# oxfordcontrol/COSMO.jl

Hardware: NVIDIA H100
Metric: ADMM iterations/sec (higher is better)
Workload: dtype f64

## Files before the change

cosmo.jl_b200/csrc/common.cuh:

```cuda
#pragma once
#include <cuda_runtime.h>
#include <stdint.h>

#include <limits>

namespace cosmo {

constexpr int kBlock = 256;
constexpr int kWarpsPerBlock = kBlock / 32;
constexpr int kMaxGrid = 132 * 8;
constexpr int kMaxRed = 8;

template <typename T>
struct CsrView {
  const int* rowptr;
  const int* col;
  const T* val;
};

template <typename T>
struct RedBuf {
  T* partials;
  T* out;
  unsigned* ticket;
// ... 39 lines not shown
}
__device__ __forceinline__ void mbar_wait(uint64_t* bar, unsigned parity) {
  const unsigned addr = (unsigned)__cvta_generic_to_shared(bar);
  asm volatile(
      "{\n\t"
      ".reg .pred p;\n\t"
      "WAIT_LOOP:\n\t"
      "mbarrier.try_wait.parity.shared::cta.b64 p, [%0], %1;\n\t"
      "@p bra WAIT_DONE;\n\t"
      "bra WAIT_LOOP;\n\t"
      "WAIT_DONE:\n\t"
      "}" ::"r"(addr),
      "r"(parity)
      : "memory");
}

constexpr int kMaxRanks = 8;
template <typename T>
struct P2pView {
  T* peer_data[kMaxRanks];
  unsigned* peer_flags[kMaxRanks];
  const unsigned* local_flags;
  unsigned* seq;
  size_t stride;
  int nranks, rank;
};
__device__ __forceinline__ void st_release_sys(unsigned* p, unsigned v) {
  asm volatile("st.release.sys.global.u32 [%0], %1;" ::"l"(p), "r"(v) : "memory");
}
__device__ __forceinline__ unsigned ld_acquire_sys(const unsigned* p) {
// ... 111 lines not shown
```

cosmo.jl_b200/csrc/engine.cu:

```cuda
#include <cuda_runtime.h>
#include <dlfcn.h>
#include <math.h>
#include <stdio.h>
#include <stdlib.h>
#include <string.h>

#include <algorithm>
#include <functional>
#include <thread>
#include <chrono>
#include <string>
#include <vector>

#include "../../include/cosmo_b200.h"
#include "common.cuh"
#include "host.cuh"
#include "psd.cuh"
#include "cone3.cuh"
#include "aa.cuh"
#include "spmv.cuh"
#include "vector_kernels.cuh"
#include "ruiz.cuh"
#include "cg_persistent.cuh"
#include "ldl.cuh"
// ... 232 lines not shown
  std::vector<int> ldl_fptr_h_, ldl_bptr_h_;
  int ldl_N_ = 0, ldl_ws_ctas_ = 1, ldl_solve_nodes_ = 0, ldl_factor_nodes_ = 0;
  long long ldl_nnzK_ = 0, ldl_nnzL_ = 0, ldl_factorizations_ = 0;
  double ldl_symbolic_s_ = 0.0, ldl_factor_s_ = 0.0;
  DevBuf<int64_t> ldl_Kp_, ldl_Ksp_, ldl_Ksrc_, ldl_Lp_, ldl_Rp_, ldl_Rmap_;
  DevBuf<int> ldl_Ki_, ldl_Li_, ldl_Rj_, ldl_fcols_, ldl_fptr_, ldl_bcols_, ldl_bptr_, ldl_perm_, ldl_flags_;
  DevBuf<T> ldl_Kx_, ldl_Lx_, ldl_Rx_, ldl_D_, ldl_Dinv_, ldl_ws_, ldl_y_;
  GraphExec ldl_factor_graph_, ldl_solve_graph_;
  Event ldl_ev_[2];
  void ldl_setup();
  void ldl_factor();
  void ldl_solve();
  void destroy_ldl_factor_graph() { ldl_factor_graph_.reset(); }
  long long kkt_counter_ = 1;
  int last_cg_iters_ = 1;
  long long total_inner_ = 0, total_mults_ = 0;
  DevBuf<T> vec_m_, vec_n_, vec_n2_, dy_, dx_, ypart_;
  DevBuf<unsigned> chunk_ticket_;
  int num_sms_ = 132;
  DevBuf<T> sc_;
  DevBuf<int> isc_;
  DevBuf<T> partials_;
  DevBuf<unsigned> ticket_;
  PinnedBuf<T> h_sc_;
  PinnedBuf<int> h_isc_;
  cudaStream_t stream_ = nullptr;
  Event ev0_, ev1_;
  long long launches_ = 0;
  int nranks_ = 1, rank_ = 0;
  NcclComm comm_ = nullptr;
// ... 26 lines not shown
    cudaError_t e = cudaGetLastError();
    if (e != cudaSuccess) throw EngineError{COSMO_B200_ERR_CUDA, std::string("launch of ") + what + " failed: " + cudaGetErrorString(e)};
    ++launches_;
  }
  void sync() { CUDA_TRY(cudaStreamSynchronize(stream_)); }
  void upload_vec(DevBuf<T>& dst, const void* host, size_t count);
  void download_vec(void* host, const T* src, size_t count);
  void build_csr(DevCsr<T>& dst, const HostCsr& h);
  void build_windows(DevCsr<T>& dst, const HostCsr& h);
  void classify_and_set_rho(bool reset_rho, bool rebuild_vec = true);
  void allreduce_sum(T* buf, size_t count);
  void allreduce_max(T* buf, size_t count);

  template <typename Epi>
  void launch_spmv(const DevCsr<T>& M1, const T* x1, const DevCsr<T>* M2, const T* x2, int nrows, const Epi& epi,
                   RedBuf<T> rb, const char* name);
  void project_device(const T* w, bool with_rhs, const T* ws_rhs);
  void soc_norms(const T* ws, T* norm_out);
  void kkt_core(bool fused_tail, const T* w_src, T* w_dst);
  void kkt_op_stage2(const int* done, const T* u, const T* t_in, T* c_out, bool exchange = false);
  void kkt_cg(const int* done);
  void kkt_minres(bool full);
  void set_maxit(int v);
  void compute_residuals(const T* x, const T* s, const T* mu, bool ignore_scaling, double out[5]);
  bool adapt_rho(const T* x);
  bool primal_infeasible();
  bool dual_infeasible();
  double inf_rec_[8] = {0, 0, 0, 0, 0, 0, 0, 0};
  void recover_mu(const T* w_prev) {
    recover_mu_kernel<T><<<vgrid(m_), kBlock, 0, stream_>>>(m_, rho_vec_.p, w_prev + n_, s_.p, mu_.p);
    check_launch("recover_mu");
  }
  void read_scalars(int first, int count) {
    CUDA_TRY(cudaMemcpyAsync(h_sc_.p + first, sc_.p + first, count * sizeof(T), cudaMemcpyDeviceToHost, stream_));
    sync();
  }
// ... 709 lines not shown
    xv_.peer_data[r] = static_cast<T*>(pd);
    xv_.peer_flags[r] = static_cast<unsigned*>(pf);
  }
  for (int r = nranks; r < kMaxRanks; ++r) { xv_.peer_data[r] = nullptr; xv_.peer_flags[r] = nullptr; }
  xv_.local_flags = xchg_flags_.p;
  xv_.seq = xchg_seq_.p;
  xv_.nranks = nranks;
  xv_.rank = rank_;
  destroy_cg_graphs();
  p2p_ = true;
}

template <typename T>
template <typename Epi>
void Engine<T>::launch_spmv(const DevCsr<T>& M1, const T* x1, const DevCsr<T>* M2, const T* x2, int nrows,
                            const Epi& epi, RedBuf<T> rb, const char* name) {
  const CsrView<T> v2 = M2 ? M2->view() : CsrView<T>{nullptr, nullptr, nullptr};
  if (M1.windowed) {
    const size_t smem = (size_t)M1.W * sizeof(T);
    static bool configured[64] = {false};
    const int dev_slot = device_ & 63;
    if (!configured[dev_slot] || device_ >= 64) {
      CUDA_TRY(cudaFuncSetAttribute(spmv_win_kernel<T, Epi>, cudaFuncAttributeMaxDynamicSharedMemorySize, 204800));
      configured[dev_slot] = true;
    }
    spmv_win_kernel<T, Epi><<<M1.nctas, kWinThreads, smem, stream_>>>(M1.wview(), x1, v2, x2, epi, rb, ypart_.p,
                                                                      chunk_ticket_.p);
    check_launch(name);
    return;
  }
  const int lanes = M1.lanes;
  const int grid = sgrid(nrows, lanes);
  if (lanes == 32) spmv_kernel<T, 32, Epi><<<grid, kBlock, 0, stream_>>>(M1.view(), x1, v2, x2, nrows, epi, rb);
  else if (lanes == 8) spmv_kernel<T, 8, Epi><<<grid, kBlock, 0, stream_>>>(M1.view(), x1, v2, x2, nrows, epi, rb);
  else spmv_kernel<T, 2, Epi><<<grid, kBlock, 0, stream_>>>(M1.view(), x1, v2, x2, nrows, epi, rb);
  check_launch(name);
}

template <typename T>
void Engine<T>::soc_norms(const T* ws, T* norm_out) {
  if (!n_soc_) return;
  if (n_soc_chunks_) {
    soc_chunk_kernel<T><<<n_soc_chunks_, kBlock, 0, stream_>>>(ws, soc_chunk_start_.p, soc_chunk_len_.p, soc_chunk_sum_.p);
    check_launch("soc_chunk");
  }
  soc_final_kernel<T><<<(n_soc_ + 127) / 128, 128, 0, stream_>>>(soc_chunk_sum_.p, soc_cone_chunk_ptr_.p, n_soc_, norm_out);
  check_launch("soc_final");
}

template <typename T>
void Engine<T>::project_device(const T* w, bool with_rhs, const T* ws_rhs) {
// ... 10 lines not shown
  a.soc = SocTable<T>{soc_off_.p, soc_norm_.p};
  a.s = s_.p; a.ls = ls_.p; a.t0 = t0_.p; a.sigma = (T)st_.sigma;
  a.do_proj = 1; a.do_rhs = with_rhs ? 1 : 0;
  launch_proj_rhs(a);
}

template <typename T>
void Engine<T>::kkt_op_stage2(const int* done, const T* u, const T* t_in, T* c_out, bool exchange) {
  const bool lead = (rank_ == 0);
  const bool px = exchange && p2p_;
  const T sig = lead ? (T)st_.sigma : (T)0;
  const DevCsr<T>* M2 = nullptr;
  const T* pu = nullptr;
  if (At_.windowed) {
    if (lead && P_.nnz > 0) {
      launch_spmv(P_, u, (const DevCsr<T>*)nullptr, (const T*)nullptr, n_, EpiStore<T>{done, vec_n2_.p}, red(SC_TMP0), "spmv_P");
      pu = vec_n2_.p;
    }
  } else if (lead) {
    M2 = &P_;
  }
  launch_spmv(At_, t_in, M2, u, n_, EpiKktOp<T>{done, c_out, u, sig, pu}, red_ptr(cb_.p + n_), "spmv_kkt_op");
  if (px) {
    if (c_out != cb_.p) throw EngineError{COSMO_B200_ERR_INVALID, "peer exchange expects the operator output in cb_"};
    const int len = n_ + 1;
    const int gx = std::max(1, std::min(16, (len * (int)sizeof(T) + 32767) / 32768));
    p2p_push_kernel<T><<<dim3(gx, nranks_), kBlock, 0, stream_>>>(xv_, cb_.p, len, done, xchg_arrive_.p);
    check_launch("p2p_push");
  }
}

template <typename T>
void Engine<T>::set_maxit(int v) {
  if (cur_maxit_ == v) return;
  h_isc_[ISC_MAXIT] = v;
  CUDA_TRY(cudaMemcpyAsync(isc_.p + ISC_MAXIT, h_isc_.p + ISC_MAXIT, sizeof(int), cudaMemcpyHostToDevice, stream_));
  sync();
  cur_maxit_ = v;
}

template <typename T>
void Engine<T>::kkt_core(bool fused_tail, const T* w_src, T* w_dst) {
  const bool lead = (rank_ == 0);
  const bool full = (st_.kkt_solver == COSMO_B200_KKT_MINRES);
  const bool direct = (st_.kkt_solver == COSMO_B200_KKT_LDL);
  if (st_.kkt_solver != COSMO_B200_KKT_CG && st_.kkt_solver != COSMO_B200_KKT_MINRES_REDUCED && !full && !direct)
    throw EngineError{COSMO_B200_ERR_UNSUPPORTED, "unknown kkt_solver"};
  if (full && nranks_ > 1)
    throw EngineError{COSMO_B200_ERR_UNSUPPORTED, "full-KKT MINRES is single-GPU in this build (use CG or reduced MINRES when sharded)"};
  if (full || direct) {
    if (direct) ldl_solve();
    else kkt_minres(true);
    if (fused_tail) {
      admm_tail_kernel<T><<<vgrid(m_), kBlock, 0, stream_>>>(m_, nu_.p, rho_vec_.p, s_.p, w_src + n_, w_dst + n_, (T)st_.alpha);
      check_launch("admm_tail");
    }
    return;
  }
  launch_spmv(At_, t0_.p, (const DevCsr<T>*)nullptr, (const T*)nullptr, n_,
              EpiAddVec<T>{nullptr, rhsb_.p, lead ? ls_.p : nullptr}, red(SC_TMP0), "spmv_rhs");
  allreduce_sum(rhsb_.p, n_);
  if (st_.kkt_solver == COSMO_B200_KKT_CG) kkt_cg(isc_.p + ISC_DONE);
  else kkt_minres(false);
  kkt_counter_ += 1;
  if (fused_tail) {
    launch_spmv(A_, xsol_.p, (const DevCsr<T>*)nullptr, (const T*)nullptr, m_,
                EpiAdmmTail<T>{nullptr, ls_.p + n_, rho_vec_.p, s_.p, w_src + n_, w_dst + n_, (T)st_.alpha}, red(SC_TMP0),
                "spmv_admm_tail");
  } else {
    launch_spmv(A_, xsol_.p, (const DevCsr<T>*)nullptr, (const T*)nullptr, m_,
                EpiY2<T>{nullptr, nu_.p, ls_.p + n_, rho_vec_.p}, red(SC_TMP0), "spmv_y2");
  }
}

template <typename T>
void Engine<T>::kkt_cg(const int* done) {
  set_maxit(n_);
  if (persistent_cg_ok()) {
    launch_persistent_cg(st_.tol_constant / pow((double)kkt_counter_, st_.tol_exponent));
    return;
  }
  launch_spmv(A_, xsol_.p, (const DevCsr<T>*)nullptr, (const T*)nullptr, m_, EpiScale<T>{nullptr, tm_.p, rho_vec_.p},
              red(SC_TMP0), "spmv_A_scale");
  kkt_op_stage2(nullptr, xsol_.p, tm_.p, cb_.p, true);
  if (!p2p_) allreduce_sum(cb_.p, n_ + 1);
  const double tol_num = st_.tol_constant / pow((double)kkt_counter_, st_.tol_exponent);
  cg_init_kernel<T><<<vgrid(n_), kBlock, 0, stream_>>>(n_, rhsb_.p, cb_.p, r_.p, u_.p, red(SC_RES2),
                                                      CgInitFin<T>{sc_.p, isc_.p, (T)tol_num, p2p_ ? xchg_seq_.p : nullptr}, p2p_, xv_);
  check_launch("cg_init");
  if (!cg_graph_[0]) build_cg_graphs(done);
  int chunk = std::max(last_cg_iters_, 0);
  for (;;) {
    int left = chunk;
    for (int b = 3; b >= 0; --b)
      while (left >= (1 << b)) {
        CUDA_TRY(cudaGraphLaunch(cg_graph_[b], stream_));
        launches_ += (long long)(1 << b) * (At_.windowed && P_.nnz > 0 ? 5 : 4);
        left -= (1 << b);
      }
    CUDA_TRY(cudaMemcpyAsync(h_isc_.p, isc_.p, 2 * sizeof(int), cudaMemcpyDeviceToHost, stream_));
    sync();
    if (h_isc_[ISC_DONE]) break;
    chunk = 1;
  }
  const int iters = h_isc_[ISC_IT];
  last_cg_iters_ = iters;
  total_inner_ += iters;
  total_mults_ += 1 + iters;
}

template <typename T>
bool Engine<T>::persistent_cg_ok() {
// ... 25 lines not shown
  a.A = A_.view(); a.At = At_.view(); a.P = P_.view();
  a.n = n_; a.m = m_;
  a.rhs = rhsb_.p; a.rho = rho_vec_.p; a.x = xsol_.p; a.r = r_.p; a.u = u_.p; a.tm = tm_.p; a.c = cb_.p;
  a.partA = persist_part_.p; a.partB = persist_part_.p + (size_t)persist_grid_ * 2;
  a.sc = sc_.p; a.isc = isc_.p; a.sigma = (T)st_.sigma; a.tol_num = (T)tol_num;
  void* args[] = {&a};
  const void* fn = persist_lanes_ == 32 ? (const void*)cg_persistent_kernel<T, 32>
                 : persist_lanes_ == 8 ? (const void*)cg_persistent_kernel<T, 8> : (const void*)cg_persistent_kernel<T, 2>;
  CUDA_TRY(cudaLaunchCooperativeKernel(fn, dim3(persist_grid_), dim3(kBlock), args, 0, stream_));
  check_launch("cg_persistent");
  ++persist_solves_;
}

template <typename T>
void Engine<T>::cg_iteration_launches(const int* done) {
  cg_update_u_kernel<T><<<vgrid(n_), kBlock, 0, stream_>>>(n_, r_.p, u_.p, sc_.p, isc_.p);
  check_launch("cg_update_u");
  launch_spmv(A_, u_.p, (const DevCsr<T>*)nullptr, (const T*)nullptr, m_, EpiScale<T>{done, tm_.p, rho_vec_.p}, red(SC_TMP0),
              "spmv_A_scale");
  kkt_op_stage2(done, u_.p, tm_.p, cb_.p, true);
  if (!p2p_) allreduce_sum(cb_.p, n_ + 1);
  cg_update_xr_kernel<T><<<vgrid(n_), kBlock, 0, stream_>>>(n_, u_.p, cb_.p, cb_.p + n_, xsol_.p, r_.p, sc_.p, isc_.p, red(SC_RES2),
                                                         CgStepFin<T>{sc_.p, isc_.p, p2p_ ? xchg_seq_.p : nullptr}, p2p_, xv_);
  check_launch("cg_update_xr");
}

template <typename T>
void Engine<T>::build_cg_graphs(const int* done) {
  cg_iteration_launches(done);
  sync();
  const long long saved = launches_;
  for (int b = 0; b < 4; ++b)
    capture_graph(cg_graph_[b], stream_, [&] { for (int i = 0; i < (1 << b); ++i) cg_iteration_launches(done); });
  launches_ = saved;
}

template <typename T>
void Engine<T>::kkt_minres(bool full) {
// ... 86 lines not shown
  out[2] = nmax(nmax(m1, m2), m3);
  out[3] = nmax(nmax(d1, d2), d3);
  out[4] = (1.0 / c_) * (0.5 * xPx + qx);
}

template <typename T>
bool Engine<T>::adapt_rho(const T* x) {
  double r[5];
  compute_residuals(x, s_.p, mu_.p, true, r);
  double rp = r[0] / (r[2] + 1e-10);
  double rd = r[1] / (r[3] + 1e-10);
  double new_rho = rho_ * sqrt(rp / (rd + 1e-10));
  new_rho = std::min(std::max(new_rho, st_.RHO_MIN), st_.RHO_MAX);
  if (new_rho > st_.adaptive_rho_tolerance * rho_ || new_rho < (1.0 / st_.adaptive_rho_tolerance) * rho_) {
    rho_ = new_rho;
    rho_vec_kernel<T><<<vgrid(m_), kBlock, 0, stream_>>>(m_, rho_class_.p, (T)rho_, (T)st_.RHO_EQ_OVER_RHO_INEQ, (T)st_.RHO_MIN, rho_vec_.p);
    check_launch("rho_vec");
    ldl_dirty_ = true;
    rho_updates_.push_back(new_rho);
    return true;
  }
  return false;
}

template <typename T>
bool Engine<T>::primal_infeasible() {
  const T eps = (T)st_.eps_prim_inf;
  double* rec = inf_rec_;
  for (int k = 0; k < 8; ++k) rec[k] = (k == 0 || k >= 6) ? 0.0 : NAN;
  rec[1] = 1;
// ... 276 lines not shown

template <typename T>
void Engine<T>::accelerator_stats(int64_t* out) {
  out[0] = aa_accelerated_; out[1] = aa_declined_; out[2] = aa_rejected_;
  out[3] = aa_rho_restarts_; out[4] = aa_mem_restarts_; out[5] = aa_activated_at_;
}

template <typename T>
void Engine<T>::solve(cosmo_b200_result* out) {
  const double t_start = now_s();
  CUDA_TRY(cudaSetDevice(device_));
  const int n = n_, m = m_;
  const long long launches0 = launches_;
  total_inner_ = 0; total_mults_ = 0;
  persist_solves_ = 0;
  CUDA_TRY(cudaMemsetAsync(isc_.p + ISC_TOTAL, 0, sizeof(int), stream_));
  int status = COSMO_B200_UNDETERMINED;
  double cost = INFINITY;
  double info[5] = {INFINITY, INFINITY, 0.0, 0.0, INFINITY};
  long long iter = 0;
  bool rho_update_due = false, infeasibility_check_due = false;
  double res_time = 0.0;

  cur_ = 0; prev_ = 1;
  CUDA_TRY(cudaMemcpyAsync(W_[cur_].p, xs_.p, n * sizeof(T), cudaMemcpyDeviceToDevice, stream_));
  ws_from_mu_kernel<T><<<vgrid(m), kBlock, 0, stream_>>>(m, rho_vec_.p, mu_.p, s_.p, W_[cur_].p + n);
  check_launch("ws_from_mu");
  is_optimized_ = true;
  {
    const bool timers = (st_.verbose & 2) != 0 || (long long)n + m >= 20000 || !psd_.large_h.empty();
// ... 198 lines not shown
void Engine<T>::project(const void* ws, void* s_out) {
  CUDA_TRY(cudaSetDevice(device_));
  if (proj_w_.n < (size_t)n_ + m_) { proj_w_.alloc((size_t)n_ + m_); proj_s_.alloc(std::max(m_, 1), false); }
  upload_vec(vec_m_, ws, m_);
  CUDA_TRY(cudaMemcpyAsync(proj_s_.p, s_.p, m_ * sizeof(T), cudaMemcpyDeviceToDevice, stream_));
  CUDA_TRY(cudaMemcpyAsync(proj_w_.p + n_, vec_m_.p, m_ * sizeof(T), cudaMemcpyDeviceToDevice, stream_));
  project_device(proj_w_.p, false, nullptr);
  download_vec(s_out, s_.p, m_);
  CUDA_TRY(cudaMemcpyAsync(s_.p, proj_s_.p, m_ * sizeof(T), cudaMemcpyDeviceToDevice, stream_));
  sync();
}

template <typename T>
void Engine<T>::kkt_solve(const void* rhs, void* sol, int64_t* inner) {
  CUDA_TRY(cudaSetDevice(device_));
  upload_vec(ls_, rhs, (size_t)n_ + m_);
  scale_kernel<T><<<vgrid(m_), kBlock, 0, stream_>>>(m_, rho_vec_.p, ls_.p + n_, t0_.p);
  check_launch("scale_x2");
  kkt_core(false, nullptr, nullptr);
  download_vec(sol, xsol_.p, n_);
  download_vec(static_cast<T*>(sol) + n_, nu_.p, m_);
  sync();
  if (inner && st_.kkt_solver == COSMO_B200_KKT_LDL) {
    *inner = 0;
  } else if (inner) {
    CUDA_TRY(cudaMemcpyAsync(h_isc_.p, isc_.p, 2 * sizeof(int), cudaMemcpyDeviceToHost, stream_));
    sync();
    *inner = h_isc_[ISC_IT];
  }
}
// ... 152 lines not shown
template <typename T>
void Engine<T>::spmv(int which, const void* x, void* y) {
  CUDA_TRY(cudaSetDevice(device_));
  if (which == 0) {
    upload_vec(dx_, x, n_);
    launch_spmv(A_, dx_.p, (const DevCsr<T>*)nullptr, (const T*)nullptr, m_, EpiStore<T>{nullptr, vec_m_.p}, red(SC_TMP0), "spmv_A");
    download_vec(y, vec_m_.p, m_);
  } else if (which == 1) {
    upload_vec(dy_, x, m_);
    launch_spmv(At_, dy_.p, (const DevCsr<T>*)nullptr, (const T*)nullptr, n_, EpiStore<T>{nullptr, vec_n_.p}, red(SC_TMP0), "spmv_At");
    download_vec(y, vec_n_.p, n_);
  } else if (which == 2) {
    upload_vec(dx_, x, n_);
    launch_spmv(P_, dx_.p, (const DevCsr<T>*)nullptr, (const T*)nullptr, n_, EpiStore<T>{nullptr, vec_n_.p}, red(SC_TMP0), "spmv_P");
    download_vec(y, vec_n_.p, n_);
  } else {
    throw EngineError{COSMO_B200_ERR_INVALID, "spmv: which must be 0 (A), 1 (A') or 2 (P)"};
  }
  sync();
}

template <typename T>
void Engine<T>::spmv_bench(int which, int reps, double* ms, double* bytes) {
  CUDA_TRY(cudaSetDevice(device_));
  if (reps < 1) reps = 1;
  auto one = [&]() {
    if (which == 0)
      launch_spmv(A_, xsol_.p, (const DevCsr<T>*)nullptr, (const T*)nullptr, m_, EpiScale<T>{nullptr, tm_.p, rho_vec_.p}, red(SC_TMP0), "spmv_A_scale");
    else if (which == 1)
      launch_spmv(At_, tm_.p, (const DevCsr<T>*)nullptr, (const T*)nullptr, n_, EpiStore<T>{nullptr, vec_n_.p}, red(SC_TMP0), "spmv_At");
    else if (which == 2)
      launch_spmv(P_, xsol_.p, (const DevCsr<T>*)nullptr, (const T*)nullptr, n_, EpiStore<T>{nullptr, vec_n_.p}, red(SC_TMP0), "spmv_P");
// ... 286 lines not shown
```

cosmo.jl_b200/csrc/host.cuh:

```cuda
#pragma once
#include <cuda_runtime.h>
#include <stdio.h>

#include <string>
#include <vector>

#include "../../include/cosmo_b200.h"

namespace cosmo {

struct EngineError {
  int code;
  std::string msg;
};

#define CUDA_TRY(expr)                                                                              \
  do {                                                                                              \
    cudaError_t _e = (expr);                                                                        \
    if (_e != cudaSuccess) {                                                                        \
      char _b[512];                                                                                 \
      snprintf(_b, sizeof(_b), "CUDA error %s at %s:%d: %s", cudaGetErrorName(_e), __FILE__,        \
               __LINE__, cudaGetErrorString(_e));                                                   \
      throw EngineError{COSMO_B200_ERR_CUDA, _b};                                                   \
    }                                                                                               \
// ... 47 lines not shown
  cudaEvent_t e = nullptr;
  Event() {} Event(const Event&) = delete; Event& operator=(const Event&) = delete;
  ~Event() { if (e) cudaEventDestroy(e); }
  void create() { if (!e) CUDA_TRY(cudaEventCreate(&e)); }
  operator cudaEvent_t() const { return e; }
};

struct GraphExec {
  cudaGraphExec_t g = nullptr;
  GraphExec() {} GraphExec(const GraphExec&) = delete; GraphExec& operator=(const GraphExec&) = delete;
  ~GraphExec() { reset(); }
  void reset() { if (g) cudaGraphExecDestroy(g); g = nullptr; }
  operator cudaGraphExec_t() const { return g; }
};

template <typename F>
void capture_graph(GraphExec& out, cudaStream_t st, F&& launches) {
  out.reset();
  cudaGraph_t graph = nullptr;
  CUDA_TRY(cudaStreamBeginCapture(st, cudaStreamCaptureModeThreadLocal));
  launches();
  CUDA_TRY(cudaStreamEndCapture(st, &graph));
  CUDA_TRY(cudaGraphInstantiate(&out.g, graph, 0));
  CUDA_TRY(cudaGraphDestroy(graph));
}

}
```

cosmo.jl_b200/csrc/spmv.cuh:

```cuda
#pragma once
#include "common.cuh"

namespace cosmo {

template <typename T, bool NC>
__device__ __forceinline__ T gather_ld(const T* p) {
  if (NC) return __ldg(p);
  return __ldcg(p);
}

template <typename T, int LANES, bool NC = true>
__device__ __forceinline__ T row_partial(const CsrView<T>& M, const T* __restrict__ x, int row, int lane) {
  const int start = __ldg(M.rowptr + row);
  const int end = __ldg(M.rowptr + row + 1);
  T s0 = 0, s1 = 0;
  if (LANES == 32) {
    int a0 = (start + 3) & ~3;
    if (a0 > end) a0 = end;
    {
      const int i = start + lane;
      if (i < a0) s0 += __ldcs(M.val + i) * gather_ld<T, NC>(x + __ldcs(M.col + i));
    }
    const int body_end = a0 + ((end - a0) & ~3);
#pragma unroll 2
// ... 14 lines not shown
    for (int j = start + lane; j < end; j += LANES) s0 += __ldcs(M.val + j) * gather_ld<T, NC>(x + __ldcs(M.col + j));
  }
  return s0 + s1;
}

template <typename T, int LANES>
__device__ __forceinline__ T group_sum(T v) {
#pragma unroll
  for (int o = LANES / 2; o > 0; o >>= 1) v += __shfl_xor_sync(0xffffffffu, v, o, LANES);
  return v;
}

template <typename T, int LANES, typename Epi>
__global__ void __launch_bounds__(kBlock) spmv_kernel(CsrView<T> M1, const T* __restrict__ x1, CsrView<T> M2,
                                                      const T* __restrict__ x2, int nrows, Epi epi, RedBuf<T> rb) {
  if (epi.done != nullptr && *epi.done) return;
  constexpr int GROUPS = kBlock / LANES;
  const int lane = threadIdx.x % LANES;
  const int group = threadIdx.x / LANES;
  const int total_groups = gridDim.x * GROUPS;
  T accS[Epi::NS > 0 ? Epi::NS : 1];
  T accM[Epi::NM > 0 ? Epi::NM : 1];
#pragma unroll
  for (int k = 0; k < (Epi::NS > 0 ? Epi::NS : 1); ++k) accS[k] = 0;
#pragma unroll
  for (int k = 0; k < (Epi::NM > 0 ? Epi::NM : 1); ++k) accM[k] = 0;

  for (int base = blockIdx.x * GROUPS; base < nrows; base += total_groups) {
    const int row = base + group;
    const bool valid = row < nrows;
// ... 39 lines not shown
__device__ __forceinline__ T win_row_rest(const unsigned short* __restrict__ col, const T* __restrict__ val, const T* xs,
                                          int start, int end, int lane) {
  T s = 0;
  for (int j0 = start + 256; j0 < end; j0 += 256) {
    const int L = min(32, (end - j0) >> 3);
    if (lane < L) {
      const uint4 c = __ldcs(reinterpret_cast<const uint4*>(col + j0 + lane * 8));
      T v[8];
      load8_coalesced(val + j0, L, lane, v);
      s += win_fma8<T>(v, c, xs);
    }
  }
  return s;
}

template <typename T, typename Epi>
__global__ void __launch_bounds__(kWinThreads, 1) spmv_win_kernel(WcsrView<T> M, const T* __restrict__ x, CsrView<T> M2,
                                                                  const T* __restrict__ x2, Epi epi, RedBuf<T> rb,
                                                                  T* __restrict__ ypart, unsigned* __restrict__ chunk_ticket) {
  if (epi.done != nullptr && *epi.done) return;
  extern __shared__ __align__(128) unsigned char win_smem[];
  T* xs = reinterpret_cast<T*>(win_smem);
  __shared__ __align__(8) uint64_t bar;
  __shared__ int fin_flag;
  const int lane = threadIdx.x & 31, warp = threadIdx.x >> 5;
  const int w = blockIdx.x % M.nwin, chunk = blockIdx.x / M.nwin;
  const int nchunks = gridDim.x / M.nwin;
  if (threadIdx.x == 0) {
    mbar_init(&bar, 1);
    mbar_fence_init();
    int cnt = M.ncols - w * M.W;
    if (cnt > M.W) cnt = M.W;
    const unsigned bytes = ((unsigned)cnt * (unsigned)sizeof(T) + 15u) & ~15u;
    mbar_expect_tx(&bar, bytes);
    bulk_load_g2s(xs, x + (size_t)w * M.W, bytes, &bar);
  }
  __syncthreads();
  const int r0 = M.cta_row_start[chunk], r1 = M.cta_row_start[chunk + 1];
  T accS[Epi::NS > 0 ? Epi::NS : 1];
  T accM[Epi::NM > 0 ? Epi::NM : 1];
#pragma unroll
  for (int k = 0; k < (Epi::NS > 0 ? Epi::NS : 1); ++k) accS[k] = 0;
#pragma unroll
  for (int k = 0; k < (Epi::NM > 0 ? Epi::NM : 1); ++k) accM[k] = 0;

  const int* rp = M.rowptr + (size_t)w * (M.nrows + 1);
  const bool single = (M.nwin == 1);
  T* yw = ypart + (size_t)w * M.nrows;
  const int nmine = (r1 - r0 - warp + kWinWarps - 1) / kWinWarps;
  bool waited = false;
  int sa = 0, ea = 0, sb = 0, eb = 0;
  auto fetch_ptrs = [&](int k, int& s_a, int& e_a, int& s_b, int& e_b) {
    s_a = e_a = s_b = e_b = 0;
    if (k < nmine) {
      const int row = r0 + warp + k * kWinWarps;
      s_a = __ldg(rp + row);
      e_a = __ldg(rp + row + 1);
    }
    if (k + 1 < nmine) {
      const int row = r0 + warp + (k + 1) * kWinWarps;
      s_b = __ldg(rp + row);
      e_b = __ldg(rp + row + 1);
    }
  };
  fetch_ptrs(0, sa, ea, sb, eb);
  for (int k = 0; k < nmine; k += 2) {
    const bool has_b = (k + 1 < nmine);
    const int ja = sa + lane * 8, jb = sb + lane * 8;
    const bool la = ja < ea, lb = jb < eb;
    uint4 cxa = make_uint4(0, 0, 0, 0), cxb = make_uint4(0, 0, 0, 0);
    T va[8], vb[8];
#pragma unroll
    for (int i = 0; i < 8; ++i) { va[i] = T(0); vb[i] = T(0); }
    if (la) { cxa = __ldcs(reinterpret_cast<const uint4*>(M.col + ja)); load8_coalesced(M.val + sa, min(32, (ea - sa) >> 3), lane, va); }
    if (lb) { cxb = __ldcs(reinterpret_cast<const uint4*>(M.col + jb)); load8_coalesced(M.val + sb, min(32, (eb - sb) >> 3), lane, vb); }
    const int csa = sa, cea = ea, csb = sb, ceb = eb;
    fetch_ptrs(k + 2, sa, ea, sb, eb);
    if (!waited) { mbar_wait(&bar, 0); waited = true; }
    T pa = la ? win_fma8<T>(va, cxa, xs) : T(0);
    T pb = lb ? win_fma8<T>(vb, cxb, xs) : T(0);
    if (cea - csa > 256) pa += win_row_rest<T>(M.col, M.val, xs, csa, cea, lane);
    if (ceb - csb > 256) pb += win_row_rest<T>(M.col, M.val, xs, csb, ceb, lane);
    const int rowa = r0 + warp + k * kWinWarps;
    const int rowb = rowa + kWinWarps;
    const bool hi = (lane & 16) != 0;
    T keep = hi ? pb : pa;
    const T send = hi ? pa : pb;
    keep += __shfl_xor_sync(0xffffffffu, send, 16);
#pragma unroll
    for (int o = 8; o > 0; o >>= 1) keep += __shfl_xor_sync(0xffffffffu, keep, o);
    if (lane == 0 || (lane == 16 && has_b)) {
      const int row = hi ? rowb : rowa;
      if (single) epi.row(row, keep, accS, accM);
      else yw[row] = keep;
    }
  }
  if (!waited) mbar_wait(&bar, 0);

  if (!single) {
    __threadfence();
    __syncthreads();
    if (threadIdx.x == 0) {
      const unsigned t = atomicAdd(chunk_ticket + chunk, 1u);
      fin_flag = (t == (unsigned)M.nwin - 1u);
      if (fin_flag) chunk_ticket[chunk] = 0u;
    }
    __syncthreads();
    if (!fin_flag) return;
    __threadfence();
    for (int row = r0 + (int)threadIdx.x; row < r1; row += kWinThreads) {
      T tot = __ldcg(ypart + row);
      for (int ww = 1; ww < M.nwin; ++ww) tot += __ldcg(ypart + (size_t)ww * M.nrows + row);
// ... 23 lines not shown
  const T* rho;
  __device__ void row(int r, T s, T*, T*) const { y[r] = rho[r] * s; }
  __device__ void operator()(T*) const {}
};

template <typename T>
struct EpiKktOp {
  static constexpr int NS = 1, NM = 0;
  const int* done;
  T* c;
  const T* u;
  T sigma;
  const T* add;
  __device__ void row(int r, T s, T* accS, T*) const {
    const T ur = u[r];
    const T v = (add ? s + add[r] : s) + sigma * ur;
    c[r] = v;
    accS[0] += ur * v;
  }
  __device__ void operator()(T*) const {}
};

template <typename T>
struct EpiAddVec {
  static constexpr int NS = 0, NM = 0;
  const int* done;
  T* y;
  const T* add;
  __device__ void row(int r, T s, T*, T*) const { y[r] = add ? s + add[r] : s; }
  __device__ void operator()(T*) const {}
};
// ... 18 lines not shown
  const T* rho;
  __device__ void row(int r, T s, T*, T*) const { y[r] = s - x2[r] / rho[r]; }
  __device__ void operator()(T*) const {}
};

template <typename T>
struct EpiAdmmTail {
  static constexpr int NS = 0, NM = 0;
  const int* done;
  const T* x2;
  const T* rho;
  const T* s;
  const T* ws_in;
  T* ws_out;
  T alpha;
  __device__ void row(int r, T sum, T*, T*) const {
    const T rh = rho[r];
    const T nu = rh * (sum - x2[r]);
    const T sr = s[r], w = ws_in[r];
    const T s_tl = T(2) * sr - w - nu / rh;
    ws_out[r] = w + alpha * (s_tl - sr);
  }
  __device__ void operator()(T*) const {}
};

template <typename T>
struct EpiPrimalRes {
  static constexpr int NS = 0, NM = 4;
  const int* done;
  const T* s;
  const T* b;
  const T* Einv;
// ... 50 lines not shown
```

cosmo.jl_b200/csrc/vector_kernels.cuh:

```cuda
#pragma once
#include "common.cuh"

namespace cosmo {

enum {
  SC_RES = 0,
  SC_PREV = 1,
  SC_TOL = 2,
  SC_RES2 = 3,
  SC_RHS2 = 4,
  SC_TMP0 = 5,
  SC_TMP1 = 6,
  SC_TMP2 = 7,
  SC_TMP3 = 8,
  SC_TMP4 = 9,
  SC_TMP5 = 10,
  SC_TMP6 = 11,
  SC_TMP7 = 12,
  SC_H1 = 16, SC_H2 = 17, SC_H3 = 18, SC_H4 = 19,
  SC_RHS_1 = 20, SC_RHS_2 = 21,
  SC_C_PREV = 22, SC_S_PREV = 23, SC_C_CURR = 24, SC_S_CURR = 25,
  SC_K3_INV_H4 = 26, SC_K3_H2 = 27, SC_K3_H1 = 28, SC_K3_INV_H3 = 29, SC_K3_RHS1 = 30,
  SC_COUNT = 32
};
// ... 276 lines not shown
    const T rhsn = sqrt(out[1]);
    const T tol = tol_num / rhsn;
    sc[SC_RES] = res;
    sc[SC_PREV] = T(1);
    sc[SC_TOL] = tol;
    isc[ISC_IT] = 0;
    isc[ISC_DONE] = (res <= tol || isc[ISC_MAXIT] <= 0) ? 1 : 0;
    if (seq) *seq = *seq + 1u;
  }
};

template <typename T>
__global__ void __launch_bounds__(kBlock) cg_init_kernel(int n, const T* __restrict__ rhs, const T* __restrict__ c,
                                                         T* __restrict__ r, T* __restrict__ u, RedBuf<T> rb,
                                                         CgInitFin<T> fin, bool p2p, P2pView<T> xv) {
  T accS[2] = {0, 0};
  T accM[1] = {0};
  unsigned slot = 0;
  if (p2p) {
    const unsigned sq = *xv.seq;
    slot = sq & 1u;
    p2p_wait_all(xv, slot, sq + 1u);
  }
  for (int i = blockIdx.x * blockDim.x + threadIdx.x; i < n; i += gridDim.x * blockDim.x) {
    const T b = rhs[i];
    const T ci = p2p ? p2p_gather(xv, slot, i) : c[i];
    const T ri = b - ci;
    r[i] = ri;
    u[i] = T(0);
    accS[0] += ri * ri;
    accS[1] += b * b;
  }
  reduce_and_finalize<T, 2, 0>(accS, accM, rb, fin);
}

template <typename T>
__global__ void __launch_bounds__(kBlock) cg_update_u_kernel(int n, const T* __restrict__ r, T* __restrict__ u,
                                                             const T* __restrict__ sc, const int* __restrict__ isc) {
  if (isc[ISC_DONE]) return;
  const T res = sc[SC_RES], prev = sc[SC_PREV];
  const T beta = (res * res) / (prev * prev);
  for (int i = blockIdx.x * blockDim.x + threadIdx.x; i < n; i += gridDim.x * blockDim.x) u[i] = r[i] + beta * u[i];
}

template <typename T>
struct CgStepFin {
  T* sc; int* isc;
  unsigned* seq;
  __device__ void operator()(T* out) const {
    const T res = sqrt(out[0]);
    sc[SC_PREV] = sc[SC_RES];
    sc[SC_RES] = res;
    const int it = isc[ISC_IT] + 1;
    isc[ISC_IT] = it;
    isc[ISC_DONE] = (res <= sc[SC_TOL] || it >= isc[ISC_MAXIT]) ? 1 : 0;
    if (seq) *seq = *seq + 1u;
  }
};

template <typename T>
__global__ void __launch_bounds__(kBlock) cg_update_xr_kernel(int n, const T* __restrict__ u, const T* __restrict__ c,
                                                              const T* __restrict__ dot_uc, T* __restrict__ x,
                                                              T* __restrict__ r, const T* __restrict__ sc,
                                                              const int* __restrict__ isc, RedBuf<T> rb,
                                                              CgStepFin<T> fin, bool p2p, P2pView<T> xv) {
  if (isc[ISC_DONE]) return;
  const T res = sc[SC_RES];
  unsigned slot = 0;
  T dot;
  if (p2p) {
    const unsigned sq = *xv.seq;
    slot = sq & 1u;
    p2p_wait_all(xv, slot, sq + 1u);
    dot = p2p_gather(xv, slot, n);
  } else {
    dot = dot_uc[0];
  }
  const T alpha = (res * res) / dot;
  T accS[1] = {0};
  T accM[1] = {0};
// ... 223 lines not shown
```

cosmo.jl_b200/engine.py:

```python
from __future__ import annotations

import ctypes as C
import os
from typing import Optional, Sequence

import numpy as np

from . import build as _build

OK = 0
ERR_INVALID, ERR_UNSUPPORTED, ERR_CUDA, ERR_ALLOC, ERR_NCCL, ERR_NUMERICAL = -1, -2, -3, -4, -5, -6
F64, F32 = 0, 1
ZERO, NONNEG, BOX, SOC, PSD_SQUARE, PSD_TRIANGLE, EXP, DUAL_EXP, POW, DUAL_POW, PSD_TRIANGLE_COMPLEX = range(11)
STATUS = {0: "Undetermined", 1: "Solved", 2: "Max_iter_reached", 3: "Time_limit_reached",
          4: "Primal_infeasible", 5: "Dual_infeasible", 6: "Unsolved"}
KKT_CG, KKT_MINRES_REDUCED, KKT_MINRES, KKT_LDL = 0, 1, 2, 3
ACC_EMPTY, ACC_ANDERSON = 0, 1
AA_TYPE2_QR, AA_TYPE2_NORMAL, AA_TYPE1 = 0, 1, 2
AA_RESTARTED_MEMORY, AA_ROLLING_MEMORY = 0, 1
AA_NO_REGULARIZER, AA_TIKONOV, AA_FROBENIUS = 0, 1, 2
AA_IMMEDIATE, AA_ITER, AA_ACCURACY = 0, 1, 2


class EngineError(RuntimeError):
# ... 315 lines not shown

    def kkt_solve(self, rhs):
        rhs = self._vec(rhs, self.n + self.m)
        sol = np.empty(self.n + self.m, dtype=self.dtype)
        inner = C.c_int64(0)
        self._check(self._lib.cosmo_b200_kkt_solve(self._h, _ptr(rhs), _ptr(sol), C.byref(inner)))
        return sol, inner.value

    def residuals(self, x, s, mu, ignore_scaling=False):
        x, s, mu = self._vec(x, self.n), self._vec(s, self.m), self._vec(mu, self.m)
        out = (C.c_double * 5)()
        self._check(self._lib.cosmo_b200_residuals(self._h, _ptr(x), _ptr(s), _ptr(mu), int(ignore_scaling), out))
        return tuple(out)

    def spmv(self, which, x):
        size_in = self.m if which == 1 else self.n
        size_out = self.m if which == 0 else self.n
        x = self._vec(x, size_in)
        y = np.empty(size_out, dtype=self.dtype)
        self._check(self._lib.cosmo_b200_spmv(self._h, which, _ptr(x), _ptr(y)))
        return y

    def spmv_bench(self, which, reps=20):
        ms, nbytes = C.c_double(0), C.c_double(0)
        self._check(self._lib.cosmo_b200_spmv_bench(self._h, which, reps, C.byref(ms), C.byref(nbytes)))
        return ms.value, nbytes.value

    def rho_vec(self):
        out = np.empty(self.m, dtype=self.dtype)
        self._check(self._lib.cosmo_b200_get_rho_vec(self._h, _ptr(out)))
        return out
# ... 98 lines not shown
```

Measured before the change: 43.41.

## Add PDL launches, fold P SpMV into windowed kernel, reuse tail tm

Launches the CG, SpMV and vector kernels with programmatic dependent launch so a kernel's prologue (barrier init, row pointer prefetch) overlaps the previous kernel's tail. When P is plain CSR it is folded into the windowed A' SpMV kernel via a pbuf, which removes a separate P SpMV launch per CG iteration. The ADMM tail epilogue now stores rho*A*x into tm so the next KKT solve can skip its initial A-scale SpMV, with invalidation on rho changes and fresh solves. It also adds a which=3 KKT-operator SpMV test entry point. The risks are added complexity around cached-state validity and PDL ordering.

Result: faster. 45.31, median of 6 (+4.4%).

```diff
diff --git a/cosmo.jl_b200/csrc/common.cuh b/cosmo.jl_b200/csrc/common.cuh
--- a/cosmo.jl_b200/csrc/common.cuh
+++ b/cosmo.jl_b200/csrc/common.cuh
@@ -77,6 +77,9 @@
       "r"(parity)
       : "memory");
 }
+
+__device__ __forceinline__ void pdl_launch_dependents() { asm volatile("griddepcontrol.launch_dependents;" ::: "memory"); }
+__device__ __forceinline__ void pdl_wait() { asm volatile("griddepcontrol.wait;" ::: "memory"); }
 
 constexpr int kMaxRanks = 8;
 template <typename T>
diff --git a/cosmo.jl_b200/csrc/engine.cu b/cosmo.jl_b200/csrc/engine.cu
--- a/cosmo.jl_b200/csrc/engine.cu
+++ b/cosmo.jl_b200/csrc/engine.cu
@@ -270,6 +270,7 @@
   void destroy_ldl_factor_graph() { ldl_factor_graph_.reset(); }
   long long kkt_counter_ = 1;
   int last_cg_iters_ = 1;
+  bool tm_valid_ = false;
   long long total_inner_ = 0, total_mults_ = 0;
   DevBuf<T> vec_m_, vec_n_, vec_n2_, dy_, dx_, ypart_;
   DevBuf<unsigned> chunk_ticket_;
@@ -326,12 +327,14 @@
 
   template <typename Epi>
   void launch_spmv(const DevCsr<T>& M1, const T* x1, const DevCsr<T>* M2, const T* x2, int nrows, const Epi& epi,
-                   RedBuf<T> rb, const char* name);
+                   RedBuf<T> rb, const char* name, T* pbuf = nullptr);
+  template <typename Epi, int PL>
+  void launch_win(const DevCsr<T>& M1, const T* x1, CsrView<T> v2, const T* x2, const Epi& epi, RedBuf<T> rb, T* pbuf);
   void project_device(const T* w, bool with_rhs, const T* ws_rhs);
   void soc_norms(const T* ws, T* norm_out);
   void kkt_core(bool fused_tail, const T* w_src, T* w_dst);
   void kkt_op_stage2(const int* done, const T* u, const T* t_in, T* c_out, bool exchange = false);
-  void kkt_cg(const int* done);
+  void kkt_cg(const int* done, bool tm_ready);
   void kkt_minres(bool full);
   void set_maxit(int v);
   void compute_residuals(const T* x, const T* s, const T* mu, bool ignore_scaling, double out[5]);
@@ -1071,27 +1074,42 @@
 template <typename T>
 template <typename Epi>
 void Engine<T>::launch_spmv(const DevCsr<T>& M1, const T* x1, const DevCsr<T>* M2, const T* x2, int nrows,
-                            const Epi& epi, RedBuf<T> rb, const char* name) {
+                            const Epi& epi, RedBuf<T> rb, const char* name, T* pbuf) {
   const CsrView<T> v2 = M2 ? M2->view() : CsrView<T>{nullptr, nullptr, nullptr};
   if (M1.windowed) {
-    const size_t smem = (size_t)M1.W * sizeof(T);
-    static bool configured[64] = {false};
-    const int dev_slot = device_ & 63;
-    if (!configured[dev_slot] || device_ >= 64) {
-      CUDA_TRY(cudaFuncSetAttribute(spmv_win_kernel<T, Epi>, cudaFuncAttributeMaxDynamicSharedMemorySize, 204800));
-      configured[dev_slot] = true;
-    }
-    spmv_win_kernel<T, Epi><<<M1.nctas, kWinThreads, smem, stream_>>>(M1.wview(), x1, v2, x2, epi, rb, ypart_.p,
-                                                                      chunk_ticket_.p);
+    if (M2 == nullptr) {
+      launch_win<Epi, 0>(M1, x1, v2, x2, epi, rb, nullptr);
+    } else if constexpr (std::is_same<Epi, EpiKktOp<T>>::value) {
+      if (M2->windowed || pbuf == nullptr) throw EngineError{COSMO_B200_ERR_INVALID, "windowed SpMV: P rows need plain CSR and a buffer"};
+      if (M2->lanes == 32) launch_win<Epi, 32>(M1, x1, v2, x2, epi, rb, pbuf);
+      else if (M2->lanes == 8) launch_win<Epi, 8>(M1, x1, v2, x2, epi, rb, pbuf);
+      else launch_win<Epi, 2>(M1, x1, v2, x2, epi, rb, pbuf);
+    } else {
+      throw EngineError{COSMO_B200_ERR_INVALID, "windowed SpMV: a second matrix is only folded into the KKT operator"};
+    }
     check_launch(name);
     return;
   }
   const int lanes = M1.lanes;
   const int grid = sgrid(nrows, lanes);
-  if (lanes == 32) spmv_kernel<T, 32, Epi><<<grid, kBlock, 0, stream_>>>(M1.view(), x1, v2, x2, nrows, epi, rb);
-  else if (lanes == 8) spmv_kernel<T, 8, Epi><<<grid, kBlock, 0, stream_>>>(M1.view(), x1, v2, x2, nrows, epi, rb);
-  else spmv_kernel<T, 2, Epi><<<grid, kBlock, 0, stream_>>>(M1.view(), x1, v2, x2, nrows, epi, rb);
+  auto kernel = lanes == 32 ? spmv_kernel<T, 32, Epi> : lanes == 8 ? spmv_kernel<T, 8, Epi> : spmv_kernel<T, 2, Epi>;
+  launch_pdl(kernel, grid, kBlock, 0, stream_, M1.view(), x1, v2, x2, nrows, epi, rb);
   check_launch(name);
+}
+
+template <typename T>
+template <typename Epi, int PL>
+void Engine<T>::launch_win(const DevCsr<T>& M1, const T* x1, CsrView<T> v2, const T* x2, const Epi& epi, RedBuf<T> rb,
+                           T* pbuf) {
+  const size_t smem = (size_t)M1.W * sizeof(T);
+  static bool configured[64] = {false};
+  const int dev_slot = device_ & 63;
+  if (!configured[dev_slot] || device_ >= 64) {
+    CUDA_TRY(cudaFuncSetAttribute(spmv_win_kernel<T, Epi, PL>, cudaFuncAttributeMaxDynamicSharedMemorySize, 204800));
+    configured[dev_slot] = true;
+  }
+  launch_pdl(spmv_win_kernel<T, Epi, PL>, M1.nctas, kWinThreads, smem, stream_, M1.wview(), x1, v2, x2, epi, rb, ypart_.p,
+             chunk_ticket_.p, pbuf);
 }
 
 template <typename T>
@@ -1132,13 +1150,16 @@
   const T* pu = nullptr;
   if (At_.windowed) {
     if (lead && P_.nnz > 0) {
-      launch_spmv(P_, u, (const DevCsr<T>*)nullptr, (const T*)nullptr, n_, EpiStore<T>{done, vec_n2_.p}, red(SC_TMP0), "spmv_P");
       pu = vec_n2_.p;
+      if (P_.windowed)
+        launch_spmv(P_, u, (const DevCsr<T>*)nullptr, (const T*)nullptr, n_, EpiStore<T>{done, vec_n2_.p}, red(SC_TMP0), "spmv_P");
+      else
+        M2 = &P_;
     }
   } else if (lead) {
     M2 = &P_;
   }
-  launch_spmv(At_, t_in, M2, u, n_, EpiKktOp<T>{done, c_out, u, sig, pu}, red_ptr(cb_.p + n_), "spmv_kkt_op");
+  launch_spmv(At_, t_in, M2, u, n_, EpiKktOp<T>{done, c_out, u, sig, pu}, red_ptr(cb_.p + n_), "spmv_kkt_op", vec_n2_.p);
   if (px) {
     if (c_out != cb_.p) throw EngineError{COSMO_B200_ERR_INVALID, "peer exchange expects the operator output in cb_"};
     const int len = n_ + 1;
@@ -1166,6 +1187,8 @@
     throw EngineError{COSMO_B200_ERR_UNSUPPORTED, "unknown kkt_solver"};
   if (full && nranks_ > 1)
     throw EngineError{COSMO_B200_ERR_UNSUPPORTED, "full-KKT MINRES is single-GPU in this build (use CG or reduced MINRES when sharded)"};
+  const bool tm_ready = tm_valid_;
+  tm_valid_ = false;
   if (full || direct) {
     if (direct) ldl_solve();
     else kkt_minres(true);
@@ -1178,13 +1201,17 @@
   launch_spmv(At_, t0_.p, (const DevCsr<T>*)nullptr, (const T*)nullptr, n_,
               EpiAddVec<T>{nullptr, rhsb_.p, lead ? ls_.p : nullptr}, red(SC_TMP0), "spmv_rhs");
   allreduce_sum(rhsb_.p, n_);
-  if (st_.kkt_solver == COSMO_B200_KKT_CG) kkt_cg(isc_.p + ISC_DONE);
+  const bool cg = (st_.kkt_solver == COSMO_B200_KKT_CG);
+  if (cg) kkt_cg(isc_.p + ISC_DONE, tm_ready);
   else kkt_minres(false);
   kkt_counter_ += 1;
   if (fused_tail) {
+    const bool keep_tm = cg && !persistent_cg_ok();
     launch_spmv(A_, xsol_.p, (const DevCsr<T>*)nullptr, (const T*)nullptr, m_,
-                EpiAdmmTail<T>{nullptr, ls_.p + n_, rho_vec_.p, s_.p, w_src + n_, w_dst + n_, (T)st_.alpha}, red(SC_TMP0),
-                "spmv_admm_tail");
+                EpiAdmmTail<T>{nullptr, ls_.p + n_, rho_vec_.p, s_.p, w_src + n_, w_dst + n_, (T)st_.alpha,
+                               keep_tm ? tm_.p : nullptr},
+                red(SC_TMP0), "spmv_admm_tail");
+    tm_valid_ = keep_tm;
   } else {
     launch_spmv(A_, xsol_.p, (const DevCsr<T>*)nullptr, (const T*)nullptr, m_,
                 EpiY2<T>{nullptr, nu_.p, ls_.p + n_, rho_vec_.p}, red(SC_TMP0), "spmv_y2");
@@ -1192,19 +1219,20 @@
 }
 
 template <typename T>
-void Engine<T>::kkt_cg(const int* done) {
+void Engine<T>::kkt_cg(const int* done, bool tm_ready) {
   set_maxit(n_);
   if (persistent_cg_ok()) {
     launch_persistent_cg(st_.tol_constant / pow((double)kkt_counter_, st_.tol_exponent));
     return;
   }
-  launch_spmv(A_, xsol_.p, (const DevCsr<T>*)nullptr, (const T*)nullptr, m_, EpiScale<T>{nullptr, tm_.p, rho_vec_.p},
-              red(SC_TMP0), "spmv_A_scale");
+  if (!tm_ready)
+    launch_spmv(A_, xsol_.p, (const DevCsr<T>*)nullptr, (const T*)nullptr, m_, EpiScale<T>{nullptr, tm_.p, rho_vec_.p},
+                red(SC_TMP0), "spmv_A_scale");
   kkt_op_stage2(nullptr, xsol_.p, tm_.p, cb_.p, true);
   if (!p2p_) allreduce_sum(cb_.p, n_ + 1);
   const double tol_num = st_.tol_constant / pow((double)kkt_counter_, st_.tol_exponent);
-  cg_init_kernel<T><<<vgrid(n_), kBlock, 0, stream_>>>(n_, rhsb_.p, cb_.p, r_.p, u_.p, red(SC_RES2),
-                                                      CgInitFin<T>{sc_.p, isc_.p, (T)tol_num, p2p_ ? xchg_seq_.p : nullptr}, p2p_, xv_);
+  launch_pdl(cg_init_kernel<T>, vgrid(n_), kBlock, 0, stream_, n_, (const T*)rhsb_.p, (const T*)cb_.p, r_.p, u_.p, red(SC_RES2),
+             CgInitFin<T>{sc_.p, isc_.p, (T)tol_num, p2p_ ? xchg_seq_.p : nullptr}, p2p_, xv_);
   check_launch("cg_init");
   if (!cg_graph_[0]) build_cg_graphs(done);
   int chunk = std::max(last_cg_iters_, 0);
@@ -1213,7 +1241,7 @@
     for (int b = 3; b >= 0; --b)
       while (left >= (1 << b)) {
         CUDA_TRY(cudaGraphLaunch(cg_graph_[b], stream_));
-        launches_ += (long long)(1 << b) * (At_.windowed && P_.nnz > 0 ? 5 : 4);
+        launches_ += (long long)(1 << b) * (At_.windowed && P_.windowed && P_.nnz > 0 && rank_ == 0 ? 5 : 4);
         left -= (1 << b);
       }
     CUDA_TRY(cudaMemcpyAsync(h_isc_.p, isc_.p, 2 * sizeof(int), cudaMemcpyDeviceToHost, stream_));
@@ -1269,14 +1297,15 @@
 
 template <typename T>
 void Engine<T>::cg_iteration_launches(const int* done) {
-  cg_update_u_kernel<T><<<vgrid(n_), kBlock, 0, stream_>>>(n_, r_.p, u_.p, sc_.p, isc_.p);
+  launch_pdl(cg_update_u_kernel<T>, vgrid(n_), kBlock, 0, stream_, n_, (const T*)r_.p, u_.p, (const T*)sc_.p, (const int*)isc_.p);
   check_launch("cg_update_u");
   launch_spmv(A_, u_.p, (const DevCsr<T>*)nullptr, (const T*)nullptr, m_, EpiScale<T>{done, tm_.p, rho_vec_.p}, red(SC_TMP0),
               "spmv_A_scale");
   kkt_op_stage2(done, u_.p, tm_.p, cb_.p, true);
   if (!p2p_) allreduce_sum(cb_.p, n_ + 1);
-  cg_update_xr_kernel<T><<<vgrid(n_), kBlock, 0, stream_>>>(n_, u_.p, cb_.p, cb_.p + n_, xsol_.p, r_.p, sc_.p, isc_.p, red(SC_RES2),
-                                                         CgStepFin<T>{sc_.p, isc_.p, p2p_ ? xchg_seq_.p : nullptr}, p2p_, xv_);
+  launch_pdl(cg_update_xr_kernel<T>, vgrid(n_), kBlock, 0, stream_, n_, (const T*)u_.p, (const T*)cb_.p, (const T*)cb_.p + n_,
+             xsol_.p, r_.p, (const T*)sc_.p, (const int*)isc_.p, red(SC_RES2),
+             CgStepFin<T>{sc_.p, isc_.p, p2p_ ? xchg_seq_.p : nullptr}, p2p_, xv_);
   check_launch("cg_update_xr");
 }
 
@@ -1393,6 +1422,7 @@
   new_rho = std::min(std::max(new_rho, st_.RHO_MIN), st_.RHO_MAX);
   if (new_rho > st_.adaptive_rho_tolerance * rho_ || new_rho < (1.0 / st_.adaptive_rho_tolerance) * rho_) {
     rho_ = new_rho;
+    tm_valid_ = false;
     rho_vec_kernel<T><<<vgrid(m_), kBlock, 0, stream_>>>(m_, rho_class_.p, (T)rho_, (T)st_.RHO_EQ_OVER_RHO_INEQ, (T)st_.RHO_MIN, rho_vec_.p);
     check_launch("rho_vec");
     ldl_dirty_ = true;
@@ -1699,6 +1729,7 @@
   const long long launches0 = launches_;
   total_inner_ = 0; total_mults_ = 0;
   persist_solves_ = 0;
+  tm_valid_ = false;
   CUDA_TRY(cudaMemsetAsync(isc_.p + ISC_TOTAL, 0, sizeof(int), stream_));
   int status = COSMO_B200_UNDETERMINED;
   double cost = INFINITY;
@@ -1927,6 +1958,7 @@
 template <typename T>
 void Engine<T>::kkt_solve(const void* rhs, void* sol, int64_t* inner) {
   CUDA_TRY(cudaSetDevice(device_));
+  tm_valid_ = false;
   upload_vec(ls_, rhs, (size_t)n_ + m_);
   scale_kernel<T><<<vgrid(m_), kBlock, 0, stream_>>>(m_, rho_vec_.p, ls_.p + n_, t0_.p);
   check_launch("scale_x2");
@@ -2109,8 +2141,13 @@
     upload_vec(dx_, x, n_);
     launch_spmv(P_, dx_.p, (const DevCsr<T>*)nullptr, (const T*)nullptr, n_, EpiStore<T>{nullptr, vec_n_.p}, red(SC_TMP0), "spmv_P");
     download_vec(y, vec_n_.p, n_);
+  } else if (which == 3) {
+    upload_vec(dx_, x, n_);
+    upload_vec(dy_, static_cast<const T*>(x) + n_, m_);
+    kkt_op_stage2(nullptr, dx_.p, dy_.p, vec_n_.p);
+    download_vec(y, vec_n_.p, n_);
   } else {
-    throw EngineError{COSMO_B200_ERR_INVALID, "spmv: which must be 0 (A), 1 (A') or 2 (P)"};
+    throw EngineError{COSMO_B200_ERR_INVALID, "spmv: which must be 0 (A), 1 (A'), 2 (P) or 3 (A' x2 + P x1 + sigma x1)"};
   }
   sync();
 }
diff --git a/cosmo.jl_b200/csrc/host.cuh b/cosmo.jl_b200/csrc/host.cuh
--- a/cosmo.jl_b200/csrc/host.cuh
+++ b/cosmo.jl_b200/csrc/host.cuh
@@ -3,6 +3,7 @@
 #include <stdio.h>
 
 #include <string>
+#include <utility>
 #include <vector>
 
 #include "../../include/cosmo_b200.h"
@@ -85,6 +86,21 @@
   operator cudaGraphExec_t() const { return g; }
 };
 
+template <typename... KArgs, typename... Args>
+void launch_pdl(void (*kernel)(KArgs...), dim3 grid, dim3 block, size_t smem, cudaStream_t st, Args&&... args) {
+  cudaLaunchAttribute attr[1];
+  attr[0].id = cudaLaunchAttributeProgrammaticStreamSerialization;
+  attr[0].val.programmaticStreamSerializationAllowed = 1;
+  cudaLaunchConfig_t cfg = {};
+  cfg.gridDim = grid;
+  cfg.blockDim = block;
+  cfg.dynamicSmemBytes = smem;
+  cfg.stream = st;
+  cfg.attrs = attr;
+  cfg.numAttrs = 1;
+  CUDA_TRY(cudaLaunchKernelEx(&cfg, kernel, std::forward<Args>(args)...));
+}
+
 template <typename F>
 void capture_graph(GraphExec& out, cudaStream_t st, F&& launches) {
   out.reset();
diff --git a/cosmo.jl_b200/csrc/spmv.cuh b/cosmo.jl_b200/csrc/spmv.cuh
--- a/cosmo.jl_b200/csrc/spmv.cuh
+++ b/cosmo.jl_b200/csrc/spmv.cuh
@@ -52,6 +52,8 @@
 template <typename T, int LANES, typename Epi>
 __global__ void __launch_bounds__(kBlock) spmv_kernel(CsrView<T> M1, const T* __restrict__ x1, CsrView<T> M2,
                                                       const T* __restrict__ x2, int nrows, Epi epi, RedBuf<T> rb) {
+  pdl_launch_dependents();
+  pdl_wait();
   if (epi.done != nullptr && *epi.done) return;
   constexpr int GROUPS = kBlock / LANES;
   const int lane = threadIdx.x % LANES;
@@ -121,11 +123,12 @@
   return s;
 }
 
-template <typename T, typename Epi>
+template <typename T, typename Epi, int PL = 0>
 __global__ void __launch_bounds__(kWinThreads, 1) spmv_win_kernel(WcsrView<T> M, const T* __restrict__ x, CsrView<T> M2,
                                                                   const T* __restrict__ x2, Epi epi, RedBuf<T> rb,
-                                                                  T* __restrict__ ypart, unsigned* __restrict__ chunk_ticket) {
-  if (epi.done != nullptr && *epi.done) return;
+                                                                  T* __restrict__ ypart, unsigned* __restrict__ chunk_ticket,
+                                                                  T* pbuf) {
+  pdl_launch_dependents();
   extern __shared__ __align__(128) unsigned char win_smem[];
   T* xs = reinterpret_cast<T*>(win_smem);
   __shared__ __align__(8) uint64_t bar;
@@ -136,13 +139,20 @@
   if (threadIdx.x == 0) {
     mbar_init(&bar, 1);
     mbar_fence_init();
-    int cnt = M.ncols - w * M.W;
-    if (cnt > M.W) cnt = M.W;
-    const unsigned bytes = ((unsigned)cnt * (unsigned)sizeof(T) + 15u) & ~15u;
-    mbar_expect_tx(&bar, bytes);
-    bulk_load_g2s(xs, x + (size_t)w * M.W, bytes, &bar);
   }
   __syncthreads();
+  auto stage_x = [&]() -> bool {
+    pdl_wait();
+    if (epi.done != nullptr && *epi.done) return false;
+    if (threadIdx.x == 0) {
+      int cnt = M.ncols - w * M.W;
+      if (cnt > M.W) cnt = M.W;
+      const unsigned bytes = ((unsigned)cnt * (unsigned)sizeof(T) + 15u) & ~15u;
+      mbar_expect_tx(&bar, bytes);
+      bulk_load_g2s(xs, x + (size_t)w * M.W, bytes, &bar);
+    }
+    return true;
+  };
   const int r0 = M.cta_row_start[chunk], r1 = M.cta_row_start[chunk + 1];
   T accS[Epi::NS > 0 ? Epi::NS : 1];
   T accM[Epi::NM > 0 ? Epi::NM : 1];
@@ -170,7 +180,28 @@
       e_b = __ldg(rp + row + 1);
     }
   };
+  auto p_rows = [&]() {
+    constexpr int G = kWinThreads / (PL > 0 ? PL : 1);
+    const int plane = threadIdx.x % (PL > 0 ? PL : 1), group = threadIdx.x / (PL > 0 ? PL : 1);
+    for (int base = r0 + w * G; base < r1; base += M.nwin * G) {
+      const int row = base + group;
+      const bool valid = row < r1;
+      T s = 0;
+      if (valid) s += row_partial<T, (PL > 0 ? PL : 1)>(M2, x2, row, plane);
+      s = group_sum<T, (PL > 0 ? PL : 1)>(s);
+      if (valid && plane == 0) pbuf[row] = s;
+    }
+  };
   fetch_ptrs(0, sa, ea, sb, eb);
+  bool staged = false;
+  if constexpr (PL > 0) {
+    if (single) {
+      if (!stage_x()) return;
+      staged = true;
+      p_rows();
+      __syncthreads();
+    }
+  }
   for (int k = 0; k < nmine; k += 2) {
     const bool has_b = (k + 1 < nmine);
     const int ja = sa + lane * 8, jb = sb + lane * 8;
@@ -183,7 +214,11 @@
     if (lb) { cxb = __ldcs(reinterpret_cast<const uint4*>(M.col + jb)); load8_coalesced(M.val + sb, min(32, (eb - sb) >> 3), lane, vb); }
     const int csa = sa, cea = ea, csb = sb, ceb = eb;
     fetch_ptrs(k + 2, sa, ea, sb, eb);
-    if (!waited) { mbar_wait(&bar, 0); waited = true; }
+    if (!waited) {
+      if (!staged && !stage_x()) return;
+      mbar_wait(&bar, 0);
+      waited = true;
+    }
     T pa = la ? win_fma8<T>(va, cxa, xs) : T(0);
     T pb = lb ? win_fma8<T>(vb, cxb, xs) : T(0);
     if (cea - csa > 256) pa += win_row_rest<T>(M.col, M.val, xs, csa, cea, lane);
@@ -202,7 +237,13 @@
       else yw[row] = keep;
     }
   }
-  if (!waited) mbar_wait(&bar, 0);
+  if (!waited) {
+    if (!staged && !stage_x()) return;
+    mbar_wait(&bar, 0);
+  }
+  if constexpr (PL > 0) {
+    if (!single) p_rows();
+  }
 
   if (!single) {
     __threadfence();
@@ -256,7 +297,7 @@
   const T* add;
   __device__ void row(int r, T s, T* accS, T*) const {
     const T ur = u[r];
-    const T v = (add ? s + add[r] : s) + sigma * ur;
+    const T v = (add ? s + __ldcg(add + r) : s) + sigma * ur;
     c[r] = v;
     accS[0] += ur * v;
   }
@@ -305,8 +346,10 @@
   const T* ws_in;
   T* ws_out;
   T alpha;
+  T* tm;
   __device__ void row(int r, T sum, T*, T*) const {
     const T rh = rho[r];
+    if (tm) tm[r] = rh * sum;
     const T nu = rh * (sum - x2[r]);
     const T sr = s[r], w = ws_in[r];
     const T s_tl = T(2) * sr - w - nu / rh;
diff --git a/cosmo.jl_b200/csrc/vector_kernels.cuh b/cosmo.jl_b200/csrc/vector_kernels.cuh
--- a/cosmo.jl_b200/csrc/vector_kernels.cuh
+++ b/cosmo.jl_b200/csrc/vector_kernels.cuh
@@ -314,6 +314,8 @@
 __global__ void __launch_bounds__(kBlock) cg_init_kernel(int n, const T* __restrict__ rhs, const T* __restrict__ c,
                                                          T* __restrict__ r, T* __restrict__ u, RedBuf<T> rb,
                                                          CgInitFin<T> fin, bool p2p, P2pView<T> xv) {
+  pdl_launch_dependents();
+  pdl_wait();
   T accS[2] = {0, 0};
   T accM[1] = {0};
   unsigned slot = 0;
@@ -337,6 +339,8 @@
 template <typename T>
 __global__ void __launch_bounds__(kBlock) cg_update_u_kernel(int n, const T* __restrict__ r, T* __restrict__ u,
                                                              const T* __restrict__ sc, const int* __restrict__ isc) {
+  pdl_launch_dependents();
+  pdl_wait();
   if (isc[ISC_DONE]) return;
   const T res = sc[SC_RES], prev = sc[SC_PREV];
   const T beta = (res * res) / (prev * prev);
@@ -364,6 +368,8 @@
                                                               T* __restrict__ r, const T* __restrict__ sc,
                                                               const int* __restrict__ isc, RedBuf<T> rb,
                                                               CgStepFin<T> fin, bool p2p, P2pView<T> xv) {
+  pdl_launch_dependents();
+  pdl_wait();
   if (isc[ISC_DONE]) return;
   const T res = sc[SC_RES];
   unsigned slot = 0;
diff --git a/cosmo.jl_b200/engine.py b/cosmo.jl_b200/engine.py
--- a/cosmo.jl_b200/engine.py
+++ b/cosmo.jl_b200/engine.py
@@ -353,7 +353,7 @@
         return tuple(out)
 
     def spmv(self, which, x):
-        size_in = self.m if which == 1 else self.n
+        size_in = self.m if which == 1 else self.n + self.m if which == 3 else self.n
         size_out = self.m if which == 0 else self.n
         x = self._vec(x, size_in)
         y = np.empty(size_out, dtype=self.dtype)
```
